# surrealdb/surrealdb

Measured on NVIDIA H100. Metric: KNN queries/sec @recall@10=1.0 (exact brute force), higher is better.
Workload: dtype s8 screen + f64 exact

## Files before the change

### surrealdb_b200/csrc/screen_tc.cu

```cuda
#include <cuda.h>

#include <type_traits>

#include "internal.cuh"

namespace sdb {

namespace tc {
constexpr uint32_t BLOCK_M = 128;
constexpr uint32_t BLOCK_N = 256;
constexpr uint32_t BLOCK_K = 64;
constexpr uint32_t WG_M = 64;
constexpr uint32_t STAGES = 4;
constexpr uint32_t A_BYTES = BLOCK_M * BLOCK_K * 2;
constexpr uint32_t B_BYTES = BLOCK_N * BLOCK_K * 2;
constexpr uint32_t STAGE_BYTES = A_BYTES + B_BYTES;
constexpr uint32_t CONS_WARPS = 8;
constexpr uint32_t PROD_WARP = CONS_WARPS;
constexpr uint32_t DRAIN_WARP = CONS_WARPS + 2;
constexpr uint32_t MAX_MBLOCKS = 16;
constexpr uint32_t SUBCAP = 16;
constexpr uint32_t SMEM_BYTES = STAGES * STAGE_BYTES + 2 * BLOCK_N * 4 + 256 + MAX_MBLOCKS * 256 * 4 + 1024;
static_assert(BLOCK_N == TILE_ROWS, "screen tile must match the pass schedule tile");
static_assert(SMEM_BYTES <= 227 * 1024, "screen CTA must fit the shared memory of one SM");
constexpr uint32_t RING = 128;
static_assert(3 * RING * 4 <= 2 * BLOCK_N * 4, "the survivor ring must fit the screening-norm buffers");
static_assert(MAX_MBLOCKS * BLOCK_M <= 0x10000 && RING <= 32 * 1024, "ring tags: 16-bit query and sequence fields");
template <bool INT8, int MODE>
constexpr bool has_drain() { return INT8 && (MODE == 1 || MODE == 2); }
template <bool INT8, int MODE>
constexpr uint32_t threads() { return (CONS_WARPS + (has_drain<INT8, MODE>() ? 3 : 2)) * 32; }

__device__ __forceinline__ uint32_t smem_u32(const void* p) { return (uint32_t)__cvta_generic_to_shared(p); }

__device__ __forceinline__ uint32_t item_mb(uint32_t w, uint32_t n_mb) { return (w % n_mb + w / n_mb) % n_mb; }

__device__ __forceinline__ void mbar_init(uint32_t bar, uint32_t count) {
  asm volatile("mbarrier.init.shared::cta.b64 [%0], %1;" ::"r"(bar), "r"(count) : "memory");
}
__device__ __forceinline__ void mbar_expect_tx(uint32_t bar, uint32_t bytes) {
  asm volatile("mbarrier.arrive.expect_tx.shared::cta.b64 _, [%0], %1;" ::"r"(bar), "r"(bytes) : "memory");
}
__device__ __forceinline__ void mbar_arrive(uint32_t bar) {
  asm volatile("mbarrier.arrive.shared::cta.b64 _, [%0];" ::"r"(bar) : "memory");
}
__device__ __forceinline__ void mbar_wait(uint32_t bar, uint32_t parity) {
  uint32_t ok;
  do {
    asm volatile(
        "{\n\t.reg .pred p;\n\t"
        "mbarrier.try_wait.parity.shared::cta.b64 p, [%1], %2;\n\t"
        "selp.u32 %0, 1, 0, p;\n\t}"
        : "=r"(ok)
        : "r"(bar), "r"(parity)
        : "memory");
  } while (!ok);
}
__device__ __forceinline__ void tma_load_2d(uint32_t dst, const CUtensorMap* map, uint32_t c0, uint32_t c1, uint32_t bar) {
  asm volatile(
      "cp.async.bulk.tensor.2d.shared::cluster.global.tile.mbarrier::complete_tx::bytes [%0], [%1, {%2, %3}], [%4];"
      ::"r"(dst), "l"(map), "r"(c0), "r"(c1), "r"(bar)
      : "memory");
}
__device__ __forceinline__ void tma_load_2d_pair(uint32_t dst, const CUtensorMap* map, uint32_t c0, uint32_t c1,
                                                 uint32_t bar) {
  asm volatile(
      "cp.async.bulk.tensor.2d.shared::cluster.global.tile.mbarrier::complete_tx::bytes.multicast::cluster"
      " [%0], [%1, {%2, %3}], [%4], %5;"
      ::"r"(dst), "l"(map), "r"(c0), "r"(c1), "r"(bar), "h"((uint16_t)0x3)
      : "memory");
}
__device__ __forceinline__ void mbar_arrive_cta(uint32_t bar, uint32_t rank) {
  uint32_t remote;
  asm volatile("mapa.shared::cluster.u32 %0, %1, %2;" : "=r"(remote) : "r"(bar), "r"(rank));
  asm volatile("mbarrier.arrive.shared::cluster.b64 _, [%0];" ::"r"(remote) : "memory");
}
__device__ __forceinline__ uint32_t cluster_ctarank() {
  uint32_t r;
  asm volatile("mov.u32 %0, %%cluster_ctarank;" : "=r"(r));
  return r;
}
__device__ __forceinline__ void cluster_sync() {
  asm volatile("barrier.cluster.arrive.release.aligned;\n\tbarrier.cluster.wait.acquire.aligned;" ::: "memory");
}

#define SDB_WG_REGS                                                                                   \
  "{%0, %1, %2, %3, %4, %5, %6, %7, %8, %9, %10, %11, %12, %13, %14, %15, "                           \
  "%16, %17, %18, %19, %20, %21, %22, %23, %24, %25, %26, %27, %28, %29, %30, %31, "                  \
  "%32, %33, %34, %35, %36, %37, %38, %39, %40, %41, %42, %43, %44, %45, %46, %47, "                  \
  "%48, %49, %50, %51, %52, %53, %54, %55, %56, %57, %58, %59, %60, %61, %62, %63, "                  \
  "%64, %65, %66, %67, %68, %69, %70, %71, %72, %73, %74, %75, %76, %77, %78, %79, "                  \
  "%80, %81, %82, %83, %84, %85, %86, %87, %88, %89, %90, %91, %92, %93, %94, %95, "                  \
  "%96, %97, %98, %99, %100, %101, %102, %103, %104, %105, %106, %107, %108, %109, %110, %111, "      \
  "%112, %113, %114, %115, %116, %117, %118, %119, %120, %121, %122, %123, %124, %125, %126, %127}"
#define SDB_WG8(C, i) C(d[i]), C(d[i + 1]), C(d[i + 2]), C(d[i + 3]), C(d[i + 4]), C(d[i + 5]), C(d[i + 6]), C(d[i + 7])
#define SDB_WG128(C)                                                                                     \
  SDB_WG8(C, 0), SDB_WG8(C, 8), SDB_WG8(C, 16), SDB_WG8(C, 24), SDB_WG8(C, 32), SDB_WG8(C, 40), SDB_WG8(C, 48), \
      SDB_WG8(C, 56), SDB_WG8(C, 64), SDB_WG8(C, 72), SDB_WG8(C, 80), SDB_WG8(C, 88), SDB_WG8(C, 96),             \
      SDB_WG8(C, 104), SDB_WG8(C, 112), SDB_WG8(C, 120)

__device__ __forceinline__ void wgmma_bf16(float (&d)[128], uint64_t a_desc, uint64_t b_desc, uint32_t acc) {
  asm volatile(
      "{\n\t.reg .pred p;\n\t"
      "setp.ne.b32 p, %130, 0;\n\t"
      "wgmma.mma_async.sync.aligned.m64n256k16.f32.bf16.bf16 " SDB_WG_REGS ", %128, %129, p, 1, 1, 0, 0;\n\t}"
      : SDB_WG128("+f")
      : "l"(a_desc), "l"(b_desc), "r"(acc));
}
__device__ __forceinline__ void wgmma_i8(uint32_t (&d)[128], uint64_t a_desc, uint64_t b_desc, uint32_t acc) {
  asm volatile(
      "{\n\t.reg .pred p;\n\t"
      "setp.ne.b32 p, %130, 0;\n\t"
      "wgmma.mma_async.sync.aligned.m64n256k32.s32.s8.s8 " SDB_WG_REGS ", %128, %129, p;\n\t}"
      : SDB_WG128("+r")
      : "l"(a_desc), "l"(b_desc), "r"(acc));
}
__device__ __forceinline__ void acc_fence(float (&d)[128]) {
#pragma unroll
  for (int i = 0; i < 128; i++) asm volatile("" : "+f"(d[i])::"memory");
}
__device__ __forceinline__ void acc_fence(uint32_t (&d)[128]) {
#pragma unroll
  for (int i = 0; i < 128; i++) asm volatile("" : "+r"(d[i])::"memory");
}
#undef SDB_WG128
#undef SDB_WG8
#undef SDB_WG_REGS
__device__ __forceinline__ void wgmma_fence() { asm volatile("wgmma.fence.sync.aligned;" ::: "memory"); }
__device__ __forceinline__ void wgmma_commit() { asm volatile("wgmma.commit_group.sync.aligned;" ::: "memory"); }
template <int N>
__device__ __forceinline__ void wgmma_wait() {
  asm volatile("wgmma.wait_group.sync.aligned %0;" ::"n"(N) : "memory");
}
__device__ __forceinline__ uint64_t make_desc(uint32_t saddr) {
  uint64_t d = 0;
  d |= (uint64_t)((saddr >> 4) & 0x3FFF);
  d |= (uint64_t)1 << 16;
  d |= (uint64_t)(1024 >> 4) << 32;
  d |= (uint64_t)1 << 62;
  return d;
}

template <typename Acc>
__device__ __forceinline__ Acc acc_at(const Acc (&acc)[128], int i, int t) {
  return acc[4 * (t >> 1) + 2 * i + (t & 1)];
}
__device__ __forceinline__ uint32_t fragment_col(int t, uint32_t col_l) { return 8 * (t >> 1) + col_l + (t & 1); }
template <typename Acc>
__device__ __forceinline__ Acc acc_at_dyn(const Acc (&acc)[128], int i, int t) {
  Acc v = acc[2 * i];
#pragma unroll
  for (int u = 1; u < 64; u++) v = u == t ? acc_at(acc, i, u) : v;
  return v;
}
__device__ __forceinline__ uint32_t ld_volatile(const uint32_t* p) { return *reinterpret_cast<const volatile uint32_t*>(p); }
__device__ __forceinline__ void st_volatile(uint32_t* p, uint32_t v) { *reinterpret_cast<volatile uint32_t*>(p) = v; }


template <int MODE>
__device__ __forceinline__ void append_survivor(float score, uint32_t q, uint32_t row, uint32_t col, uint32_t row0,
                                                float2 hpv, uint32_t* s_cnt_mb, Cand* __restrict__ cand,
                                                uint32_t* __restrict__ cand_cnt, uint32_t cap, Cand* __restrict__ sub,
                                                uint32_t* hist) {
  const uint32_t half = col >> 7;
  const uint32_t pos = atomicAdd(s_cnt_mb + half * BLOCK_M + row, 1u);
  const uint2 cd = make_uint2(__float_as_uint(score), row0 + col);
  const uint32_t n_slots = gridDim.x * 2;
  if (pos < SUBCAP) {
    *reinterpret_cast<uint2*>(sub + ((size_t)q * n_slots + blockIdx.x * 2 + half) * SUBCAP + pos) = cd;
  } else {
    const uint32_t p2 = atomicAdd(cand_cnt + q, 1u);
    if (p2 < cap) *reinterpret_cast<uint2*>(cand + (size_t)q * cap + p2) = cd;
  }
  if (MODE == 2) {
    HistParam hp;
    hp.lo = hpv.x;
    hp.inv_w0 = hpv.y;
    hp.w0 = 0.f;
    hp.margin = 0.f;
    atomicAdd(hist + (size_t)q * HIST_BINS + hist_bin(hp, score), 1u);
  }
}

__device__ __forceinline__ void push_survivors(const uint32_t (&acc)[128], int i, uint64_t hits, uint32_t q,
                                               uint32_t row0, uint32_t col_l, uint32_t lane, uint32_t* r_val,
                                               uint32_t* r_row, uint32_t* r_tag, uint32_t* s_ring_tail,
                                               const uint32_t* s_ring_head) {
  const uint32_t total = __reduce_add_sync(0xffffffffu, (uint32_t)__popcll(hits));
  if (total == 0) return;
  uint32_t base = 0;
  if (lane == 0) base = atomicAdd(s_ring_tail, total);
  base = __shfl_sync(0xffffffffu, base, 0);
  const uint32_t lt = (1u << lane) - 1;
  for (uint32_t off = 0; off < total;) {
    const uint32_t act = __ballot_sync(0xffffffffu, hits != 0);
    const uint32_t e = base + off + __popc(act & lt);
    off += __popc(act);
    while ((int)(base + off - RING - ld_volatile(s_ring_head)) > 0) {
    }
    if (hits) {
      const int t = __ffsll((long long)hits) - 1;
      hits &= hits - 1;
      const uint32_t slot = e % RING;
      r_val[slot] = acc_at_dyn(acc, i, t);
      r_row[slot] = row0 + fragment_col(t, col_l);
      __threadfence_block();
      st_volatile(r_tag + slot, e << 16 | q);
    }
  }
}

template <bool COSINE, bool INT8, int MODE>
__global__ void __launch_bounds__(threads<INT8, MODE>(), 1)
screen_tc_kernel(const __grid_constant__ CUtensorMap map_a, const __grid_constant__ CUtensorMap map_b,
                 const float* __restrict__ snorm, uint32_t k_blocks, uint32_t n_mblocks, uint32_t nq,
                 PassDesc pass, float* tau, Cand* __restrict__ cand,
                 uint32_t* __restrict__ cand_cnt, uint32_t cap, Cand* __restrict__ sub, uint32_t* __restrict__ sub_cnt,
                 uint32_t k, const HistParam* __restrict__ hparam, uint32_t* hist, float* __restrict__ probe,
                 uint32_t probe_stride, uint32_t sleep_min_ns, uint32_t sleep_max_ns, uint32_t pair) {
  extern __shared__ uint8_t smem_raw[];
  uint8_t* smem = reinterpret_cast<uint8_t*>((reinterpret_cast<uintptr_t>(smem_raw) + 1023) & ~uintptr_t(1023));
  uint8_t* smem_a = smem;
  uint8_t* smem_b = smem + STAGES * A_BYTES;
  float* s_snorm = reinterpret_cast<float*>(smem + STAGES * STAGE_BYTES);
  uint64_t* bars = reinterpret_cast<uint64_t*>(s_snorm + 2 * BLOCK_N);
  uint64_t* full_bar = bars;
  uint64_t* empty_bar = bars + STAGES;
  uint32_t* s_done = reinterpret_cast<uint32_t*>(bars + 2 * STAGES);
  uint32_t* s_ring_tail = s_done + 1;
  uint32_t* s_ring_head = s_done + 2;
  uint32_t* s_cnt = reinterpret_cast<uint32_t*>(reinterpret_cast<uint8_t*>(bars) + 256);
  uint32_t* r_val = reinterpret_cast<uint32_t*>(s_snorm);
  uint32_t* r_row = r_val + RING;
  uint32_t* r_tag = r_row + RING;
  constexpr bool DRAIN = has_drain<INT8, MODE>();

  const uint32_t warp = threadIdx.x >> 5, lane = threadIdx.x & 31;
  const bool PAIR = INT8 && MODE == 2 && pair != 0;
  const uint32_t rank = PAIR ? cluster_ctarank() : 0;
  const uint32_t n_mb = PAIR ? n_mblocks / 2 : n_mblocks;
  const uint32_t w_first = PAIR ? blockIdx.x / 2 : blockIdx.x, w_step = PAIR ? gridDim.x / 2 : gridDim.x;
  const uint32_t n_items = pass.count * n_mb;

  if (DRAIN) {
    for (uint32_t i = threadIdx.x; i < RING; i += blockDim.x) r_tag[i] = 0xFFFF0000u;
  }
  if (threadIdx.x == 0) {
    *s_ring_tail = 0;
    *s_ring_head = 0;
    asm volatile("prefetch.tensormap [%0];" ::"l"(&map_a) : "memory");
    asm volatile("prefetch.tensormap [%0];" ::"l"(&map_b) : "memory");
    for (uint32_t s = 0; s < STAGES; s++) {
      mbar_init(smem_u32(&full_bar[s]), 1);
      mbar_init(smem_u32(&empty_bar[s]), PAIR ? 2 * CONS_WARPS : CONS_WARPS);
    }
    asm volatile("fence.mbarrier_init.release.cluster;" ::: "memory");
    *s_done = 0;
  }
  for (uint32_t i = threadIdx.x; i < n_mblocks * 256; i += blockDim.x) s_cnt[i] = 0;
  __syncthreads();
  if (PAIR) cluster_sync();

  if (warp == PROD_WARP) {
    if (lane == 0) {
      uint32_t it = 0;
      for (uint32_t w = w_first; w < n_items; w += w_step) {
        const uint32_t tile = pass_tile(pass, w / n_mb);
        const uint32_t mb = PAIR ? 2 * item_mb(w, n_mb) + rank : item_mb(w, n_mb);
        for (uint32_t kb = 0; kb < k_blocks; kb++, it++) {
          const uint32_t s = it % STAGES, ph = (it / STAGES) & 1;
          mbar_wait(smem_u32(&empty_bar[s]), ph ^ 1);
          const uint32_t fb = smem_u32(&full_bar[s]);
          const uint32_t kc = kb * (INT8 ? 2 * BLOCK_K : BLOCK_K);
          mbar_expect_tx(fb, STAGE_BYTES);
          tma_load_2d(smem_u32(smem_a + s * A_BYTES), &map_a, kc, mb * BLOCK_M, fb);
          if (PAIR)
            tma_load_2d_pair(smem_u32(smem_b + s * B_BYTES + rank * (B_BYTES / 2)), &map_b, kc,
                             tile * BLOCK_N + rank * (BLOCK_N / 2), fb);
          else
            tma_load_2d(smem_u32(smem_b + s * B_BYTES), &map_b, kc, tile * BLOCK_N, fb);
        }
      }
    }
    __syncwarp();
  } else if (warp < CONS_WARPS) {
    const uint32_t ct = threadIdx.x;
    const uint32_t g = warp >> 2;
    const uint32_t row_base = g * WG_M + (warp & 3) * 16 + (lane >> 2);
    const uint32_t col_l = 2 * (lane & 3);
    constexpr bool pass0 = MODE == 0;
    using Acc = typename std::conditional<INT8, uint32_t, float>::type;
    Acc acc[128];
    uint32_t it = 0, j = 0;
    auto release = [&](uint32_t s) {
      if (lane == 0) {
        mbar_arrive(smem_u32(&empty_bar[s]));
        if (PAIR) mbar_arrive_cta(smem_u32(&empty_bar[s]), rank ^ 1);
      }
    };
    for (uint32_t w = w_first; w < n_items; w += w_step, j++) {
      const uint32_t tidx = w / n_mb;
      const uint32_t tile = pass_tile(pass, tidx);
      const uint32_t mb = PAIR ? 2 * item_mb(w, n_mb) + rank : item_mb(w, n_mb);
      const uint32_t row0 = tile * BLOCK_N;
      float my_tau[2];
      float2 my_hp[2];
#pragma unroll
      for (int i = 0; i < 2; i++) {
        const uint32_t q = mb * BLOCK_M + row_base + 8 * i;
        my_tau[i] = __int_as_float(0x7f800000);
        my_hp[i] = make_float2(0.f, 0.f);
        if (q < nq) {
          my_tau[i] = __ldcg(tau + q);
          if (MODE == 2) my_hp[i] = __ldg(reinterpret_cast<const float2*>(hparam + q));
        }
      }
      float* sn = s_snorm + (j & 1) * BLOCK_N;
      if (!INT8 || MODE == 3) {
        sn[ct] = __ldg(snorm + row0 + ct);
        asm volatile("bar.sync 1, 256;" ::: "memory");
      }

      const uint32_t a_off = g * (WG_M * 128);
      for (uint32_t kb = 0; kb < k_blocks; kb++, it++) {
        const uint32_t s = it % STAGES, ph = (it / STAGES) & 1;
        mbar_wait(smem_u32(&full_bar[s]), ph);
        const uint64_t da = make_desc(smem_u32(smem_a + s * A_BYTES + a_off));
        const uint64_t db = make_desc(smem_u32(smem_b + s * B_BYTES));
        wgmma_fence();
        acc_fence(acc);
#pragma unroll
        for (uint32_t kk = 0; kk < 4; kk++) {
          if constexpr (INT8) wgmma_i8(acc, da + 2 * kk, db + 2 * kk, (kb | kk) != 0);
          else wgmma_bf16(acc, da + 2 * kk, db + 2 * kk, (kb | kk) != 0);
        }
        wgmma_commit();
        acc_fence(acc);
        if (kb > 0) {
          wgmma_wait<1>();
          release((it - 1) % STAGES);
        }
      }
      wgmma_wait<0>();
      acc_fence(acc);
      release((it - 1) % STAGES);

      if constexpr (!INT8) {
#pragma unroll
        for (int jj = 0; jj < 32; jj++) {
          const float2 n2 = *reinterpret_cast<const float2*>(sn + 8 * jj + col_l);
#pragma unroll
          for (int i = 0; i < 2; i++) {
            float& a0 = acc[4 * jj + 2 * i];
            float& a1 = acc[4 * jj + 2 * i + 1];
            a0 = COSINE ? a0 * n2.x : fmaf(2.f, a0, -n2.x);
            a1 = COSINE ? a1 * n2.y : fmaf(2.f, a1, -n2.y);
          }
        }
      }
#pragma unroll
      for (int i = 0; i < 2; i++) {
        const uint32_t row = row_base + 8 * i;
        const uint32_t q = mb * BLOCK_M + row;
        if (MODE == 3) {
#pragma unroll
          for (int h = 0; h < 8; h++) {
            float m = __int_as_float(0xff800000);
#pragma unroll
            for (int jj = 4 * h; jj < 4 * h + 4; jj++) {
#pragma unroll
              for (int c = 0; c < 2; c++) {
                if constexpr (INT8) {
                  const float snv = sn[8 * jj + col_l + c];
                  if (snv == snv) m = fmaxf(m, __int2float_rd((int)acc[4 * jj + 2 * i + c]));
                } else {
                  m = fmaxf(m, acc[4 * jj + 2 * i + c]);
                }
              }
            }
            m = fmaxf(m, __shfl_xor_sync(0xffffffffu, m, 1));
            m = fmaxf(m, __shfl_xor_sync(0xffffffffu, m, 2));
            if ((lane & 3) == 0 && q < nq) probe[(size_t)q * probe_stride + tidx * 8 + h] = m;
          }
        } else if (pass0) {
          if (q < nq) {
            Cand* my_cand = cand + (size_t)q * cap + (size_t)tidx * BLOCK_N;
#pragma unroll
            for (int jj = 0; jj < 32; jj++) {
              const uint32_t col = 8 * jj + col_l;
              float s0, s1;
              if constexpr (INT8) {
                s0 = __int2float_rn((int)acc[4 * jj + 2 * i]);
                s1 = __int2float_rn((int)acc[4 * jj + 2 * i + 1]);
              } else {
                s0 = acc[4 * jj + 2 * i];
                s1 = acc[4 * jj + 2 * i + 1];
              }
              *reinterpret_cast<uint2*>(my_cand + col) = make_uint2(__float_as_uint(s0), row0 + col);
              *reinterpret_cast<uint2*>(my_cand + col + 1) = make_uint2(__float_as_uint(s1), row0 + col + 1);
            }
          }
        } else {
          uint32_t* s_cnt_mb = s_cnt + mb * 256;
          if constexpr (INT8) {
            const float ct_ = ceilf(my_tau[i]);
            const int tau_i = ct_ >= 2147483520.f ? 0x7fffffff : (ct_ <= -2147483520.f ? (int)0x80000000 : (int)ct_);
            int m = (int)0x80000000;
#pragma unroll
            for (int jj = 0; jj < 32; jj++) m = max(m, max((int)acc[4 * jj + 2 * i], (int)acc[4 * jj + 2 * i + 1]));
            if (__any_sync(0xffffffffu, m >= tau_i)) {
              uint64_t hits = 0;
              if (m >= tau_i) {
#pragma unroll
                for (int t = 0; t < 64; t++)
                  if ((int)acc_at(acc, i, t) >= tau_i) hits |= 1ull << t;
              }
              push_survivors(acc, i, hits, q, row0, col_l, lane, r_val, r_row, r_tag, s_ring_tail, s_ring_head);
            }
          } else {
            float m = __int_as_float(0xff800000);
#pragma unroll
            for (int jj = 0; jj < 32; jj++) m = fmaxf(m, fmaxf(acc[4 * jj + 2 * i], acc[4 * jj + 2 * i + 1]));
            if (m >= my_tau[i]) {
#pragma unroll
              for (int jj = 0; jj < 32; jj++) {
#pragma unroll
                for (int c = 0; c < 2; c++) {
                  const float v = acc[4 * jj + 2 * i + c];
                  if (v >= my_tau[i])
                    append_survivor<MODE>(v, q, row, 8 * jj + col_l + c, row0, my_hp[i], s_cnt_mb, cand, cand_cnt,
                                          cap, sub, hist);
                }
              }
            }
          }
        }
      }
    }
    if (DRAIN) {
      __syncwarp();
      __threadfence_block();
      if (lane == 0) atomicAdd(s_done, 1u);
    }
    if (MODE == 1 || MODE == 2) {
      if (DRAIN) asm volatile("bar.sync 2, 288;" ::: "memory");
      else asm volatile("bar.sync 1, 256;" ::: "memory");
      const uint32_t n_slots = gridDim.x * 2;
      const uint32_t half = ct / BLOCK_M, row = ct % BLOCK_M;
      for (uint32_t mb = 0; mb < n_mblocks; mb++) {
        const uint32_t qq = mb * BLOCK_M + row;
        if (qq < nq) sub_cnt[(size_t)qq * n_slots + blockIdx.x * 2 + half] = s_cnt[mb * 256 + half * BLOCK_M + row];
      }
    }
    __syncwarp();
    if (!DRAIN && lane == 0) atomicAdd(s_done, 1u);
  } else if (warp == DRAIN_WARP) {
    if (DRAIN) {
      uint32_t head = 0;
      for (;;) {
        const uint32_t e = head + lane, slot = e % RING;
        const uint32_t tag = ld_volatile(r_tag + slot);
        const uint32_t ready = __ballot_sync(0xffffffffu, (tag >> 16) == (e & 0xFFFFu));
        const uint32_t n = ready == 0xffffffffu ? 32 : __ffs(~ready) - 1;
        if (n == 0) {
          uint32_t fin = 0;
          if (lane == 0 && ld_volatile(s_done) == CONS_WARPS) {
            __threadfence_block();
            fin = ld_volatile(s_ring_tail) == head;
          }
          if (__shfl_sync(0xffffffffu, fin, 0)) break;
          __nanosleep(32);
          continue;
        }
        __threadfence_block();
        if (lane < n) {
          const int v = (int)r_val[slot];
          const uint32_t grow = r_row[slot], q = tag & 0xFFFFu;
          const uint32_t col = grow % BLOCK_N, row = q % BLOCK_M;
          if (v != 0 || __ldg(snorm + grow) == __ldg(snorm + grow)) {
            const float2 hpv = MODE == 2 ? __ldg(reinterpret_cast<const float2*>(hparam + q)) : make_float2(0.f, 0.f);
            append_survivor<MODE>(__int2float_rn(v), q, row, col, grow - col, hpv, s_cnt + q / BLOCK_M * 256, cand,
                                  cand_cnt, cap, sub, hist);
          }
        }
        __syncwarp();
        __threadfence_block();
        head += n;
        if (lane == 0) st_volatile(s_ring_head, head);
      }
      asm volatile("bar.sync 2, 288;" ::: "memory");
    }
  } else {
    if (MODE == 2) {
      volatile uint32_t* done = s_done;
      const uint32_t stride = gridDim.x;
      uint32_t n_own = nq > blockIdx.x ? (nq - blockIdx.x + stride - 1) / stride : 0;
      if (n_own > 32) n_own = 32;
      float my_tau = __int_as_float(0xff800000);
      if (lane < n_own) my_tau = __ldcg(tau + blockIdx.x + lane * stride);
      uint32_t sleep_ns = sleep_min_ns;
      while (*done < CONS_WARPS) {
        bool any = false;
        for (uint32_t j = 0; j < n_own; j++) {
          const uint32_t q = blockIdx.x + j * stride;
          const uint4* hq = reinterpret_cast<const uint4*>(hist + (size_t)q * HIST_BINS) + lane * 2;
          const uint4 ha = __ldcg(hq), hb = __ldcg(hq + 1);
          const uint32_t c[8] = {ha.x, ha.y, ha.z, ha.w, hb.x, hb.y, hb.z, hb.w};
          uint32_t sum = 0;
#pragma unroll
          for (int i = 0; i < 8; i++) sum += c[i];
          uint32_t incl = sum;
#pragma unroll
          for (int o = 1; o < 32; o <<= 1) {
            const uint32_t t = __shfl_down_sync(0xffffffffu, incl, o);
            if (lane + o < 32) incl += t;
          }
          const uint32_t above = incl - sum;
          const bool mine = above < k && k <= incl;
          const uint32_t who = __ballot_sync(0xffffffffu, mine);
          if (who == 0) continue;
          uint32_t bstar = 0;
          if (mine) {
            uint32_t acc = above;
#pragma unroll
            for (int i = 7; i >= 0; i--) {
              acc += c[i];
              if (acc >= k) {
                bstar = lane * 8 + i;
                break;
              }
            }
          }
          bstar = __shfl_sync(0xffffffffu, bstar, __ffs(who) - 1);
          const float4 hv = __ldg(reinterpret_cast<const float4*>(hparam + q));
          HistParam hp;
          hp.lo = hv.x;
          hp.inv_w0 = hv.y;
          hp.w0 = hv.z;
          hp.margin = hv.w;
          const double e0 = hist_edge(hp, bstar), e1 = hist_edge(hp, bstar + 1);
          const float tn = __double2float_rd(e0 - (double)hp.margin - 0.02 * (e1 - e0) - 2e-6 * fabs(e0));
          const float told = __shfl_sync(0xffffffffu, my_tau, j);
          if (tn > told) {
            if (lane == j) my_tau = tn;
            if (lane == 0) __stcg(tau + q, tn);
            any = true;
          }
        }
        sleep_ns = any ? sleep_min_ns : (sleep_ns * 2 < sleep_max_ns ? sleep_ns * 2 : sleep_max_ns);
        __nanosleep(sleep_ns);
      }
    }
  }
  __syncthreads();
  if (PAIR) cluster_sync();
}
}

typedef CUresult (*EncodeTiledFn)(CUtensorMap*, CUtensorMapDataType, cuuint32_t, void*, const cuuint64_t*,
                                  const cuuint64_t*, const cuuint32_t*, const cuuint32_t*, CUtensorMapInterleave,
                                  CUtensorMapSwizzle, CUtensorMapL2promotion, CUtensorMapFloatOOBfill);

static EncodeTiledFn get_encode(Ctx* ctx) {
  if (!ctx->encode_tiled) {
    void* fn = nullptr;
    cudaDriverEntryPointQueryResult qres;
    if (cudaGetDriverEntryPoint("cuTensorMapEncodeTiled", &fn, cudaEnableDefault, &qres) != cudaSuccess ||
        qres != cudaDriverEntryPointSuccess)
      fn = nullptr;
    ctx->encode_tiled = fn;
  }
  return reinterpret_cast<EncodeTiledFn>(ctx->encode_tiled);
}

static sdb_status make_map(Ctx* ctx, CUtensorMap* map, const void* base, uint64_t rows, uint32_t dim_pad,
                           uint32_t box_rows, bool stream_once, bool int8 = false) {
  EncodeTiledFn enc = get_encode(ctx);
  if (!enc) {
    set_error("cuTensorMapEncodeTiled driver entry point not available");
    return SDB_ECUDA;
  }
  cuuint64_t gdim[2] = {dim_pad, rows};
  cuuint64_t gstride[1] = {(cuuint64_t)dim_pad * (int8 ? 1 : 2)};
  cuuint32_t box[2] = {int8 ? 2 * tc::BLOCK_K : tc::BLOCK_K, box_rows};
  cuuint32_t estr[2] = {1, 1};
  CUresult r = enc(map, int8 ? CU_TENSOR_MAP_DATA_TYPE_UINT8 : CU_TENSOR_MAP_DATA_TYPE_BFLOAT16, 2, const_cast<void*>(base), gdim, gstride, box, estr,
                   CU_TENSOR_MAP_INTERLEAVE_NONE, CU_TENSOR_MAP_SWIZZLE_128B,
                   stream_once ? CU_TENSOR_MAP_L2_PROMOTION_L2_256B : CU_TENSOR_MAP_L2_PROMOTION_L2_128B,
                   CU_TENSOR_MAP_FLOAT_OOB_FILL_NONE);
  if (r != CUDA_SUCCESS) {
    set_error("cuTensorMapEncodeTiled failed (%d)", (int)r);
    return SDB_ECUDA;
  }
  return SDB_OK;
}

bool screen_tc_available() { return true; }

sdb_status screen_tc_init_device(Ctx* ctx) {
#define SET_SMEM(COS, I8, MODE) \
  SDB_CUDA(cudaFuncSetAttribute(tc::screen_tc_kernel<COS, I8, MODE>, cudaFuncAttributeMaxDynamicSharedMemorySize, (int)tc::SMEM_BYTES))
  SET_SMEM(true, false, 0); SET_SMEM(true, false, 1); SET_SMEM(true, false, 2); SET_SMEM(true, false, 3);
  SET_SMEM(false, false, 0); SET_SMEM(false, false, 1); SET_SMEM(false, false, 2); SET_SMEM(false, false, 3);
  SET_SMEM(true, true, 0); SET_SMEM(true, true, 1); SET_SMEM(true, true, 2); SET_SMEM(true, true, 3);
#undef SET_SMEM
  cudaLaunchConfig_t cfg = {};
  cfg.gridDim = dim3((uint32_t)ctx->sm_count & ~1u);
  cfg.blockDim = dim3(tc::threads<true, 2>());
  cfg.dynamicSmemBytes = tc::SMEM_BYTES;
  cudaLaunchAttribute attr[1];
  attr[0].id = cudaLaunchAttributeClusterDimension;
  attr[0].val.clusterDim.x = 2;
  attr[0].val.clusterDim.y = 1;
  attr[0].val.clusterDim.z = 1;
  cfg.attrs = attr;
  cfg.numAttrs = 1;
  int clusters = 0;
  SDB_CUDA(cudaOccupancyMaxActiveClusters(&clusters, tc::screen_tc_kernel<true, true, 2>, &cfg));
  ctx->tc_pair_ctas = 2 * clusters;
  return SDB_OK;
}

sdb_status screen_tc_pass(Corpus* c, uint32_t nq, uint32_t k, const PassDesc& p, bool int8, int mode, cudaStream_t st) {
  if (p.count == 0) return SDB_OK;
  Ctx* ctx = c->ctx;
  if (int8 ? (!c->d_i8 || c->metric != SDB_COSINE) : !c->d_bf16) {
    set_error("tensor-core screen: the %s screen copy is not available for this corpus", int8 ? "int8 (cosine only)" : "bf16");
    return SDB_EUNSUPPORTED;
  }
  const uint64_t n_pad = (c->n + TILE_ROWS - 1) / TILE_ROWS * TILE_ROWS;
  uint32_t sleep_min = 512, sleep_max = 8192;
  if (const char* e = getenv("SDB_REFINE_SLEEP_MIN")) sleep_min = (uint32_t)atoi(e);
  if (const char* e = getenv("SDB_REFINE_SLEEP_MAX")) sleep_max = (uint32_t)atoi(e);
  if (sleep_min < 32) sleep_min = 32;
  if (sleep_max < sleep_min) sleep_max = sleep_min;
  const uint32_t k_blocks = int8 ? c->dim_pad8 / (2 * tc::BLOCK_K) : c->dim_pad / tc::BLOCK_K;
  const uint32_t chunk_q = tc::MAX_MBLOCKS * tc::BLOCK_M;
  const uint32_t nq0 = nq < chunk_q ? nq : chunk_q;
  const uint32_t mb0 = (nq0 + tc::BLOCK_M - 1) / tc::BLOCK_M;
  const uint32_t mb_last = (nq - (nq - 1) / chunk_q * chunk_q + tc::BLOCK_M - 1) / tc::BLOCK_M;
  uint32_t grid = (uint32_t)ctx->sm_count;
  {
    const uint64_t items0 = (uint64_t)p.count * mb0;
    if (grid > items0) grid = (uint32_t)items0;
  }
  uint32_t pair = 0;
  if (int8 && mode == 2 && mb0 % 2 == 0 && mb_last % 2 == 0) {
    const uint32_t g2 = (grid < (uint32_t)ctx->tc_pair_ctas ? grid : (uint32_t)ctx->tc_pair_ctas) & ~1u;
    if (g2 >= 2) {
      grid = g2;
      pair = 1;
    }
  }
  CUtensorMap map_b;
  if (int8) SDB_TRY(make_map(ctx, &map_b, c->d_i8, n_pad, c->dim_pad8, pair ? tc::BLOCK_N / 2 : tc::BLOCK_N, true, true));
  else SDB_TRY(make_map(ctx, &map_b, c->d_bf16, n_pad, c->dim_pad, tc::BLOCK_N, true));
  if (mode == 3 && p.count * 8 > PROBE_STRIDE) {
    set_error("screen_tc_pass: probe of %u tiles exceeds the probe buffer", p.count);
    return SDB_EINVAL;
  }
  if (mode != 3) c->last_slots = grid * 2;
  const uint32_t slots = grid * 2;
  for (uint32_t q0 = 0; q0 < nq; q0 += chunk_q) {
    const uint32_t nqc = nq - q0 < chunk_q ? nq - q0 : chunk_q;
    const uint32_t nq_pad = (nqc + tc::BLOCK_M - 1) / tc::BLOCK_M * tc::BLOCK_M;
    const uint32_t n_mblocks = nq_pad / tc::BLOCK_M;
    CUtensorMap map_a;
    if (int8) SDB_TRY(make_map(ctx, &map_a, c->d_q8 + (size_t)q0 * c->dim_pad8, nq_pad, c->dim_pad8, tc::BLOCK_M, false, true));
    else SDB_TRY(make_map(ctx, &map_a, c->d_qbf16 + (size_t)q0 * c->dim_pad, nq_pad, c->dim_pad, tc::BLOCK_M, false));
    float* tau = c->d_tau + q0;
    Cand* cand = c->d_cand + (size_t)q0 * c->sc_cap;
    uint32_t* ccnt = c->d_cand_cnt + q0;
    Cand* sub = c->d_sub + (size_t)q0 * slots * tc::SUBCAP;
    uint32_t* scnt = c->d_sub_cnt + (size_t)q0 * slots;
    const HistParam* hp = c->d_hparam + q0;
    uint32_t* hist = c->d_hist + (size_t)q0 * HIST_BINS;
    cudaLaunchConfig_t cfg = {};
    cfg.gridDim = dim3(grid);
    cfg.dynamicSmemBytes = tc::SMEM_BYTES;
    cfg.stream = st;
    cudaLaunchAttribute attr[2];
    attr[0].id = cudaLaunchAttributePriority;
    attr[0].val.priority = ctx->prio_high;
    attr[1].id = cudaLaunchAttributeClusterDimension;
    attr[1].val.clusterDim.x = pair ? 2 : 1;
    attr[1].val.clusterDim.y = 1;
    attr[1].val.clusterDim.z = 1;
    cfg.attrs = attr;
    cfg.numAttrs = pair ? 2 : 1;
    float* probe_ptr = c->d_probe + (size_t)q0 * PROBE_STRIDE;
    const uint32_t probe_stride = PROBE_STRIDE, cap_arg = c->sc_cap;
    const float* snorm_arg = c->d_snorm;
#define LAUNCH_TC1(COS, I8, MODE)                                                                                    \
  do {                                                                                                               \
    cfg.blockDim = dim3(tc::threads<I8, MODE>());                                                                    \
    SDB_CUDA(cudaLaunchKernelEx(&cfg, tc::screen_tc_kernel<COS, I8, MODE>, map_a, map_b, snorm_arg, k_blocks,        \
                                n_mblocks, nqc, p, tau, cand, ccnt, cap_arg, sub, scnt, k, hp, hist, probe_ptr,      \
                                probe_stride, sleep_min, sleep_max, pair));                                          \
  } while (0)
#define LAUNCH_TC(COS, I8)                   \
  do {                                       \
    if (mode == 0) LAUNCH_TC1(COS, I8, 0);   \
    else if (mode == 1) LAUNCH_TC1(COS, I8, 1); \
    else if (mode == 2) LAUNCH_TC1(COS, I8, 2); \
    else LAUNCH_TC1(COS, I8, 3);             \
  } while (0)
    if (int8) LAUNCH_TC(true, true);
    else if (c->metric == SDB_COSINE) LAUNCH_TC(true, false);
    else LAUNCH_TC(false, false);
#undef LAUNCH_TC
#undef LAUNCH_TC1
    count_launch(ctx);
  }
  if (mode == 0) {
    SDB_TRY(cand_set_count(c, nq, p.count * TILE_ROWS, st));
    c->last_slots = 0;
  }
  SDB_CUDA(cudaGetLastError());
  return SDB_OK;
}

}
```

Baseline: 81580.

## Hand off whole passing accumulator rows to drain warp as records

The consumer warps used to extract individual survivors from accumulator fragments with a dynamic-index select and push them one at a time into a small shared ring. Now any lane whose row maximum reaches the threshold copies its full 64-value fragment row, plus a header, into a record buffer, and the drain warp does the per-element threshold test and append. The record buffer reuses the freed count and norm space, and per-CTA counters are halved when running in pair mode. This takes extraction work off the tensor-core consumers at the cost of more shared-memory traffic and a more complex sizing of the record ring.

```diff
diff --git a/surrealdb_b200/csrc/screen_tc.cu b/surrealdb_b200/csrc/screen_tc.cu
--- a/surrealdb_b200/csrc/screen_tc.cu
+++ b/surrealdb_b200/csrc/screen_tc.cu
@@ -20,12 +20,14 @@
 constexpr uint32_t DRAIN_WARP = CONS_WARPS + 2;
 constexpr uint32_t MAX_MBLOCKS = 16;
 constexpr uint32_t SUBCAP = 16;
-constexpr uint32_t SMEM_BYTES = STAGES * STAGE_BYTES + 2 * BLOCK_N * 4 + 256 + MAX_MBLOCKS * 256 * 4 + 1024;
+constexpr uint32_t CNT_BYTES = MAX_MBLOCKS * 256 * 4;
+constexpr uint32_t SNORM_BYTES = 2 * BLOCK_N * 4;
+constexpr uint32_t SMEM_BYTES = STAGES * STAGE_BYTES + CNT_BYTES + SNORM_BYTES + 256 + 1024;
 static_assert(BLOCK_N == TILE_ROWS, "screen tile must match the pass schedule tile");
 static_assert(SMEM_BYTES <= 227 * 1024, "screen CTA must fit the shared memory of one SM");
-constexpr uint32_t RING = 128;
-static_assert(3 * RING * 4 <= 2 * BLOCK_N * 4, "the survivor ring must fit the screening-norm buffers");
-static_assert(MAX_MBLOCKS * BLOCK_M <= 0x10000 && RING <= 32 * 1024, "ring tags: 16-bit query and sequence fields");
+constexpr uint32_t REC_BYTES = 16 + 64 * 4;
+static_assert(SNORM_BYTES / REC_BYTES >= 7, "the smallest record buffer (16 query blocks, one-CTA launch)");
+static_assert(MAX_MBLOCKS * BLOCK_M <= 0x10000, "record header: 16-bit query field");
 template <bool INT8, int MODE>
 constexpr bool has_drain() { return INT8 && (MODE == 1 || MODE == 2); }
 template <bool INT8, int MODE>
@@ -141,18 +143,6 @@
   return d;
 }
 
-template <typename Acc>
-__device__ __forceinline__ Acc acc_at(const Acc (&acc)[128], int i, int t) {
-  return acc[4 * (t >> 1) + 2 * i + (t & 1)];
-}
-__device__ __forceinline__ uint32_t fragment_col(int t, uint32_t col_l) { return 8 * (t >> 1) + col_l + (t & 1); }
-template <typename Acc>
-__device__ __forceinline__ Acc acc_at_dyn(const Acc (&acc)[128], int i, int t) {
-  Acc v = acc[2 * i];
-#pragma unroll
-  for (int u = 1; u < 64; u++) v = u == t ? acc_at(acc, i, u) : v;
-  return v;
-}
 __device__ __forceinline__ uint32_t ld_volatile(const uint32_t* p) { return *reinterpret_cast<const volatile uint32_t*>(p); }
 __device__ __forceinline__ void st_volatile(uint32_t* p, uint32_t v) { *reinterpret_cast<volatile uint32_t*>(p) = v; }
 
@@ -182,30 +172,33 @@
   }
 }
 
-__device__ __forceinline__ void push_survivors(const uint32_t (&acc)[128], int i, uint64_t hits, uint32_t q,
-                                               uint32_t row0, uint32_t col_l, uint32_t lane, uint32_t* r_val,
-                                               uint32_t* r_row, uint32_t* r_tag, uint32_t* s_ring_tail,
-                                               const uint32_t* s_ring_head) {
-  const uint32_t total = __reduce_add_sync(0xffffffffu, (uint32_t)__popcll(hits));
-  if (total == 0) return;
+__device__ __forceinline__ void push_records(const uint32_t (&acc)[128], int i, uint32_t pass, uint32_t q,
+                                             uint32_t row0, uint32_t col_l, int tau_i, uint32_t lane, uint32_t recs,
+                                             uint32_t rec_cap, uint32_t tail_head) {
+  const uint32_t total = __popc(pass);
   uint32_t base = 0;
-  if (lane == 0) base = atomicAdd(s_ring_tail, total);
+  if (lane == 0) asm volatile("atom.shared.add.u32 %0, [%1], %2;" : "=r"(base) : "r"(tail_head), "r"(total) : "memory");
   base = __shfl_sync(0xffffffffu, base, 0);
-  const uint32_t lt = (1u << lane) - 1;
-  for (uint32_t off = 0; off < total;) {
-    const uint32_t act = __ballot_sync(0xffffffffu, hits != 0);
-    const uint32_t e = base + off + __popc(act & lt);
-    off += __popc(act);
-    while ((int)(base + off - RING - ld_volatile(s_ring_head)) > 0) {
-    }
-    if (hits) {
-      const int t = __ffsll((long long)hits) - 1;
-      hits &= hits - 1;
-      const uint32_t slot = e % RING;
-      r_val[slot] = acc_at_dyn(acc, i, t);
-      r_row[slot] = row0 + fragment_col(t, col_l);
+  const uint32_t r = __popc(pass & ((1u << lane) - 1));
+  const bool mine = (pass >> lane) & 1;
+  for (uint32_t off = 0; off < total; off += rec_cap) {
+    const uint32_t end = min(off + rec_cap, total);
+    for (;;) {
+      uint32_t head;
+      asm volatile("ld.volatile.shared.u32 %0, [%1];" : "=r"(head) : "r"(tail_head + 4) : "memory");
+      if ((int)(base + end - rec_cap - head) <= 0) break;
+    }
+    if (mine && r >= off && r < end) {
+      const uint32_t e = base + r;
+      const uint32_t rec = recs + (e % rec_cap) * REC_BYTES;
+#pragma unroll
+      for (int j = 0; j < 32; j++)
+        asm volatile("st.volatile.shared.v2.b32 [%0], {%1, %2};" ::"r"(rec + 16 + 8 * j), "r"(acc[4 * j + 2 * i]),
+                     "r"(acc[4 * j + 2 * i + 1]) : "memory");
+      asm volatile("st.shared.v2.b32 [%0], {%1, %2};" ::"r"(rec + 8), "r"(row0), "r"(tau_i) : "memory");
+      asm volatile("st.shared.b32 [%0], %1;" ::"r"(rec + 4), "r"(col_l << 16 | q) : "memory");
       __threadfence_block();
-      st_volatile(r_tag + slot, e << 16 | q);
+      asm volatile("st.volatile.shared.b32 [%0], %1;" ::"r"(rec), "r"(e) : "memory");
     }
   }
 }
@@ -222,17 +215,15 @@
   uint8_t* smem = reinterpret_cast<uint8_t*>((reinterpret_cast<uintptr_t>(smem_raw) + 1023) & ~uintptr_t(1023));
   uint8_t* smem_a = smem;
   uint8_t* smem_b = smem + STAGES * A_BYTES;
-  float* s_snorm = reinterpret_cast<float*>(smem + STAGES * STAGE_BYTES);
+  uint32_t* s_cnt = reinterpret_cast<uint32_t*>(smem + STAGES * STAGE_BYTES);
+  float* s_snorm = reinterpret_cast<float*>(smem + STAGES * STAGE_BYTES + CNT_BYTES);
   uint64_t* bars = reinterpret_cast<uint64_t*>(s_snorm + 2 * BLOCK_N);
   uint64_t* full_bar = bars;
   uint64_t* empty_bar = bars + STAGES;
   uint32_t* s_done = reinterpret_cast<uint32_t*>(bars + 2 * STAGES);
-  uint32_t* s_ring_tail = s_done + 1;
-  uint32_t* s_ring_head = s_done + 2;
-  uint32_t* s_cnt = reinterpret_cast<uint32_t*>(reinterpret_cast<uint8_t*>(bars) + 256);
-  uint32_t* r_val = reinterpret_cast<uint32_t*>(s_snorm);
-  uint32_t* r_row = r_val + RING;
-  uint32_t* r_tag = r_row + RING;
+  uint32_t* s_rec_tail = s_done + 1;
+  uint32_t* s_rec_head = s_done + 2;
+  static_assert(sizeof(uint64_t) * 2 * STAGES + 3 * 4 <= 256, "barriers and record counters fit their 256 bytes");
   constexpr bool DRAIN = has_drain<INT8, MODE>();
 
   const uint32_t warp = threadIdx.x >> 5, lane = threadIdx.x & 31;
@@ -241,13 +232,17 @@
   const uint32_t n_mb = PAIR ? n_mblocks / 2 : n_mblocks;
   const uint32_t w_first = PAIR ? blockIdx.x / 2 : blockIdx.x, w_step = PAIR ? gridDim.x / 2 : gridDim.x;
   const uint32_t n_items = pass.count * n_mb;
+  auto cnt_block = [&](uint32_t mb) { return s_cnt + (PAIR ? mb >> 1 : mb) * 256; };
+  uint8_t* recs = reinterpret_cast<uint8_t*>(s_cnt + n_mb * 256);
+  const uint32_t rec_cap = (CNT_BYTES - n_mb * 256 * 4 + SNORM_BYTES) / REC_BYTES;
 
   if (DRAIN) {
-    for (uint32_t i = threadIdx.x; i < RING; i += blockDim.x) r_tag[i] = 0xFFFF0000u;
+    for (uint32_t i = threadIdx.x; i < rec_cap; i += blockDim.x)
+      *reinterpret_cast<uint32_t*>(recs + i * REC_BYTES) = 0xFFFFFFFFu;
   }
   if (threadIdx.x == 0) {
-    *s_ring_tail = 0;
-    *s_ring_head = 0;
+    *s_rec_tail = 0;
+    *s_rec_head = 0;
     asm volatile("prefetch.tensormap [%0];" ::"l"(&map_a) : "memory");
     asm volatile("prefetch.tensormap [%0];" ::"l"(&map_b) : "memory");
     for (uint32_t s = 0; s < STAGES; s++) {
@@ -257,7 +252,7 @@
     asm volatile("fence.mbarrier_init.release.cluster;" ::: "memory");
     *s_done = 0;
   }
-  for (uint32_t i = threadIdx.x; i < n_mblocks * 256; i += blockDim.x) s_cnt[i] = 0;
+  for (uint32_t i = threadIdx.x; i < n_mb * 256; i += blockDim.x) s_cnt[i] = 0;
   __syncthreads();
   if (PAIR) cluster_sync();
 
@@ -401,23 +396,17 @@
             }
           }
         } else {
-          uint32_t* s_cnt_mb = s_cnt + mb * 256;
           if constexpr (INT8) {
             const float ct_ = ceilf(my_tau[i]);
             const int tau_i = ct_ >= 2147483520.f ? 0x7fffffff : (ct_ <= -2147483520.f ? (int)0x80000000 : (int)ct_);
             int m = (int)0x80000000;
 #pragma unroll
             for (int jj = 0; jj < 32; jj++) m = max(m, max((int)acc[4 * jj + 2 * i], (int)acc[4 * jj + 2 * i + 1]));
-            if (__any_sync(0xffffffffu, m >= tau_i)) {
-              uint64_t hits = 0;
-              if (m >= tau_i) {
-#pragma unroll
-                for (int t = 0; t < 64; t++)
-                  if ((int)acc_at(acc, i, t) >= tau_i) hits |= 1ull << t;
-              }
-              push_survivors(acc, i, hits, q, row0, col_l, lane, r_val, r_row, r_tag, s_ring_tail, s_ring_head);
-            }
+            const uint32_t pass = __ballot_sync(0xffffffffu, m >= tau_i);
+            if (pass)
+              push_records(acc, i, pass, q, row0, col_l, tau_i, lane, smem_u32(recs), rec_cap, smem_u32(s_rec_tail));
           } else {
+            uint32_t* s_cnt_mb = cnt_block(mb);
             float m = __int_as_float(0xff800000);
 #pragma unroll
             for (int jj = 0; jj < 32; jj++) m = fmaxf(m, fmaxf(acc[4 * jj + 2 * i], acc[4 * jj + 2 * i + 1]));
@@ -449,7 +438,8 @@
       const uint32_t half = ct / BLOCK_M, row = ct % BLOCK_M;
       for (uint32_t mb = 0; mb < n_mblocks; mb++) {
         const uint32_t qq = mb * BLOCK_M + row;
-        if (qq < nq) sub_cnt[(size_t)qq * n_slots + blockIdx.x * 2 + half] = s_cnt[mb * 256 + half * BLOCK_M + row];
+        const bool own = !PAIR || (mb & 1) == rank;
+        if (qq < nq) sub_cnt[(size_t)qq * n_slots + blockIdx.x * 2 + half] = own ? cnt_block(mb)[half * BLOCK_M + row] : 0;
       }
     }
     __syncwarp();
@@ -458,15 +448,14 @@
     if (DRAIN) {
       uint32_t head = 0;
       for (;;) {
-        const uint32_t e = head + lane, slot = e % RING;
-        const uint32_t tag = ld_volatile(r_tag + slot);
-        const uint32_t ready = __ballot_sync(0xffffffffu, (tag >> 16) == (e & 0xFFFFu));
+        const uint32_t* hdr = reinterpret_cast<const uint32_t*>(recs + ((head + lane) % rec_cap) * REC_BYTES);
+        const uint32_t ready = __ballot_sync(0xffffffffu, lane < rec_cap && ld_volatile(hdr) == head + lane);
         const uint32_t n = ready == 0xffffffffu ? 32 : __ffs(~ready) - 1;
         if (n == 0) {
           uint32_t fin = 0;
           if (lane == 0 && ld_volatile(s_done) == CONS_WARPS) {
             __threadfence_block();
-            fin = ld_volatile(s_ring_tail) == head;
+            fin = ld_volatile(s_rec_tail) == head;
           }
           if (__shfl_sync(0xffffffffu, fin, 0)) break;
           __nanosleep(32);
@@ -474,19 +463,32 @@
         }
         __threadfence_block();
         if (lane < n) {
-          const int v = (int)r_val[slot];
-          const uint32_t grow = r_row[slot], q = tag & 0xFFFFu;
-          const uint32_t col = grow % BLOCK_N, row = q % BLOCK_M;
-          if (v != 0 || __ldg(snorm + grow) == __ldg(snorm + grow)) {
-            const float2 hpv = MODE == 2 ? __ldg(reinterpret_cast<const float2*>(hparam + q)) : make_float2(0.f, 0.f);
-            append_survivor<MODE>(__int2float_rn(v), q, row, col, grow - col, hpv, s_cnt + q / BLOCK_M * 256, cand,
-                                  cand_cnt, cap, sub, hist);
+          const uint4 h = *reinterpret_cast<const uint4*>(hdr);
+          const uint32_t* val = hdr + 4;
+          const int tau_i = (int)h.w;
+          uint64_t hits = 0;
+#pragma unroll
+          for (int s = 0; s < 16; s++) {
+            const uint4 v = reinterpret_cast<const uint4*>(val)[s];
+            hits |= (uint64_t)((int)v.x >= tau_i) << (4 * s) | (uint64_t)((int)v.y >= tau_i) << (4 * s + 1) |
+                    (uint64_t)((int)v.z >= tau_i) << (4 * s + 2) | (uint64_t)((int)v.w >= tau_i) << (4 * s + 3);
+          }
+          const uint32_t q = h.y & 0xFFFFu, col_l = h.y >> 16, row0 = h.z, row = q % BLOCK_M;
+          const float2 hpv = MODE == 2 ? __ldg(reinterpret_cast<const float2*>(hparam + q)) : make_float2(0.f, 0.f);
+          while (hits) {
+            const int t = __ffsll((long long)hits) - 1;
+            hits &= hits - 1;
+            const int v = (int)val[t];
+            const uint32_t col = 8 * (t >> 1) + col_l + (t & 1);
+            if (v != 0 || __ldg(snorm + row0 + col) == __ldg(snorm + row0 + col))
+              append_survivor<MODE>(__int2float_rn(v), q, row, col, row0, hpv, cnt_block(q / BLOCK_M), cand, cand_cnt,
+                                    cap, sub, hist);
           }
         }
         __syncwarp();
         __threadfence_block();
         head += n;
-        if (lane == 0) st_volatile(s_ring_head, head);
+        if (lane == 0) st_volatile(s_rec_head, head);
       }
       asm volatile("bar.sync 2, 288;" ::: "memory");
     }
```

Result: faster. 83150 (median of 6 runs) (+1.9%).
